# ml-rust/blazr

Hardware: NVIDIA B200
Metric: decode_tokens_per_s (higher is better)
Workload: dtype int8 activations x int4/6/8 weights, f64-exact accumulate -> f32

## Files before the change

### blazr_b200/csrc/formats.cuh

```cuda
#pragma once
#ifdef B200Q_HOST_CHECK
#include "hostcheck/host_shim.h"
#else
#include "common.cuh"
#endif
#ifdef __CUDACC__
#define IQ_TABLE_QUAL static __device__
#endif
#include "iq_grids.h"

namespace b200q {

struct Unit {
    uint32_t v[8];
    float a[2], b[2];
    int off[2];
};

template <class F, class = void>
struct FmtNoff { static constexpr int value = 0; };
template <class F>
struct FmtNoff<F, decltype((void)F::NOFF)> { static constexpr int value = F::NOFF; };

struct FmtMeta {
// ... 82 lines not shown
        u.a[0] = u.a[1] = __fmul_rn(d, (float)sc);
        u.b[0] = u.b[1] = __fmul_rn(dmin, (float)m);
        u.off[0] = u.off[1] = 0;
    }
#ifndef B200Q_HOST_CHECK
    static constexpr int NOFF = 5;
    __device__ __forceinline__ static void unit_offsets(int r0, int i, FmtMeta, uint32_t (&o)[NOFF]) {
        o[0] = QS + r0 * 128 + 16 * swz8(r0, i);
        o[1] = QS + (r0 + 4) * 128 + 16 * swz8(r0 + 4, i);
        o[2] = HDR + r0 * 16;
        o[3] = HDR + r0 * 16 + 4 + i;
        o[4] = HDR + r0 * 16 + 12 + (i >> 1);
    }
    template <int STEP>
    __device__ __forceinline__ static void load_unit_at(uint32_t c, const uint32_t (&o)[NOFF], int i, Unit& u, FmtMeta) {
        const uint4 w = lds128_sa(c + o[STEP]);
        const uint32_t dd = lds32_sa(c + o[2] + 64 * STEP);
        const uint32_t b1 = lds8_sa(c + o[3] + 64 * STEP), b2 = lds8_sa(c + o[4] + 64 * STEP);
        u.v[0] = w.x & 0x0F0F0F0Fu; u.v[1] = w.y & 0x0F0F0F0Fu; u.v[2] = w.z & 0x0F0F0F0Fu; u.v[3] = w.w & 0x0F0F0F0Fu;
        u.v[4] = w.x & 0xF0F0F0F0u; u.v[5] = w.y & 0xF0F0F0F0u; u.v[6] = w.z & 0xF0F0F0F0u; u.v[7] = w.w & 0xF0F0F0F0u;
        const float d = half_bits_to_float((uint16_t)(dd & 0xFFFF)), dmin = half_bits_to_float((uint16_t)(dd >> 16));
        const int sc = b1 & 63;
        const int m = (b1 >> 6) | (((b2 >> (4 * (i & 1))) & 0xF) << 2);
        u.a[0] = u.a[1] = __fmul_rn(d, (float)sc);
        u.b[0] = u.b[1] = __fmul_rn(dmin, (float)m);
        u.off[0] = u.off[1] = 0;
    }
#endif
};

struct FmtQ6K {
// ... 60 lines not shown
        u.b[0] = u.b[1] = 0.0f;
        u.off[0] = u.off[1] = 32;
    }
#ifndef B200Q_HOST_CHECK
    static constexpr int NOFF = 6;
    __device__ __forceinline__ static void unit_offsets(int r0, int i, FmtMeta, uint32_t (&o)[NOFF]) {
        o[0] = QL + r0 * 128 + 16 * swz8(r0, i);
        o[1] = QL + (r0 + 4) * 128 + 16 * swz8(r0 + 4, i);
        o[2] = QH + r0 * 64 + 16 * swz4(r0, i >> 1) + 8 * (i & 1);
        o[3] = QH + (r0 + 4) * 64 + 16 * swz4(r0 + 4, i >> 1) + 8 * (i & 1);
        o[4] = SC + r0 * 16 + 2 * i;
        o[5] = D + r0 * 2;
    }
    template <int STEP>
    __device__ __forceinline__ static void load_unit_at(uint32_t c, const uint32_t (&o)[NOFF], int, Unit& u, FmtMeta) {
        const uint4 w = lds128_sa(c + o[STEP]);
        const uint2 hq = lds64_sa(c + o[2 + STEP]);
        const uint32_t s2 = lds16_sa(c + o[4] + 64 * STEP);
        const float d = half_bits_to_float((uint16_t)lds16_sa(c + o[5] + 8 * STEP));
        const uint32_t M4 = 0x0F0F0F0Fu, MH = 0x30303030u;
        u.v[0] = (w.x & M4) | ((hq.x << 4) & MH);
        u.v[1] = (w.y & M4) | ((hq.x << 2) & MH);
        u.v[2] = (w.z & M4) | (hq.x & MH);
        u.v[3] = (w.w & M4) | ((hq.x >> 2) & MH);
        u.v[4] = ((w.x >> 4) & M4) | ((hq.y << 4) & MH);
        u.v[5] = ((w.y >> 4) & M4) | ((hq.y << 2) & MH);
        u.v[6] = ((w.z >> 4) & M4) | (hq.y & MH);
        u.v[7] = ((w.w >> 4) & M4) | ((hq.y >> 2) & MH);
        u.a[0] = __fmul_rn(d, (float)(int8_t)(s2 & 0xFF));
        u.a[1] = __fmul_rn(d, (float)(int8_t)(s2 >> 8));
        u.b[0] = u.b[1] = 0.0f;
        u.off[0] = u.off[1] = 32;
// ... 790 lines not shown
```

### blazr_b200/csrc/internal.h

```cpp
#pragma once
#include <cuda_runtime.h>
#include <stdint.h>

#include "../../include/b200q.h"

struct b200q_weight {
    int64_t N, K, N_pad, K_pad;
    int family, source, ggml_type, group_size, sub, gpc;
    int device;
    int chunk_bytes;
    int64_t T, KC;
    uint8_t* data;
    int64_t device_bytes, canonical_bytes;
    float* bias;
    int32_t* perm;
    int num_sms;
    const b200q_weight* next;
    const b200q_weight* pair;
};

struct b200q_bank {
    int E;
    b200q_weight proto;
    const uint8_t** table_dev;
// ... 8 lines not shown
                               cudaStream_t st);
cudaError_t launch_repack_awq(const uint32_t* qweight, const float* scales, const float* zeros, int64_t N_full, int64_t n0, int64_t k0,
                              const b200q_weight* w, int* err_flag, cudaStream_t st);
cudaError_t launch_repack_gptq(const uint32_t* qweight, const float* scales, const uint32_t* qzeros, const int32_t* perm, int zpo,
                               int64_t N_full, int64_t n0, int64_t k0, const b200q_weight* w, int* err_flag, cudaStream_t st);
cudaError_t launch_dequantize(const b200q_weight* w, void* out, int dtype, cudaStream_t st);
cudaError_t launch_act_quant(const void* x, int x_dtype, int64_t M, int64_t K, int64_t K_pad, int64_t ldx, const int32_t* perm, uint8_t* xq,
                             cudaStream_t st);
cudaError_t launch_act_unpack(const uint8_t* xq, int64_t M, int64_t K_pad, int8_t* q, float* d, int32_t* bsum16, cudaStream_t st);
cudaError_t launch_int_partials(const b200q_weight* w, const uint8_t* xq, int64_t M, int32_t* out, cudaStream_t st);
cudaError_t launch_to_bf16(const void* x, int x_dtype, int64_t M, int64_t K, int64_t K_pad, int64_t M_pad, int64_t ldx, const int32_t* perm,
                           void* out_bf16, cudaStream_t st);

struct MatvecPlan {
    int grid, nstages, stage_bytes, smem_bytes, mb, xhat_bytes;
};
struct FusedPrologue {
    int mode;
    const float* h_in;
    const float* delta;
    float* h_out;
    const float* norm_w;
    float eps;
    const float* gate_up;
};
cudaError_t matvec_plan(const b200q_weight* w, int64_t M, MatvecPlan* plan, int pro = 0);
size_t matvec_ws_bytes(const b200q_weight* w, int64_t M);
void set_matvec_trace(long long* dev_buf);
cudaError_t launch_l2_prefetch(const b200q_weight* w, int64_t M, int64_t max_bytes, cudaStream_t st);
struct RemoteOut;
// ... 19 lines not shown
```

### blazr_b200/csrc/matvec.cu

```cuda
#include <cstdlib>

#include "matvec_common.cuh"

namespace b200q {

__global__ void __launch_bounds__(32) l2_prefetch_kernel(const uint8_t* __restrict__ w, int64_t KC, int64_t C, int chunk_bytes, int first, int nchunks) {
    pdl_launch_dependents();
    if (threadIdx.x != 0) return;
    const int64_t G = gridDim.x, g = blockIdx.x;
    const int64_t c0 = sk_begin(g, C, G), c1 = sk_begin(g + 1, C, G);
    const SkPlan sp = sk_plan(c0, c1, KC);
    const int n = (int)(c1 - c0);
    const uint8_t* base = w + c0 * (int64_t)chunk_bytes;
    for (int j = first; j < n && j < first + nchunks; j++) {
        const uint8_t* src;
        if (j < sp.nH) src = base + (size_t)j * chunk_bytes;
        else if (j < sp.nH + sp.nT) src = base + (size_t)(sp.nH + sp.nF + (j - sp.nH)) * chunk_bytes;
        else src = base + (size_t)(sp.nH + (j - sp.nH - sp.nT)) * chunk_bytes;
        asm volatile("cp.async.bulk.prefetch.L2.global [%0], %1;" ::"l"(src), "r"(chunk_bytes) : "memory");
    }
}


static cudaError_t launch_family(int family, const MatvecParams& p, int mb, int grid, int smem, cudaStream_t st) {
// ... 26 lines not shown
    const int cbmax = (w2 && w2->chunk_bytes > w->chunk_bytes) ? w2->chunk_bytes : w->chunk_bytes;
    int stage = cbmax + (pro ? 0 : (int)M * ACT_REC_BYTES);
    stage = (stage + 127) & ~127;
    int xhat = pro ? (int)(((size_t)w->KC * M * ACT_REC_BYTES + 127) & ~(size_t)127) : 0;
    int budget_kb = 150;
    if (const char* e = getenv("B200Q_MV_SMEM_KB")) { int v = atoi(e); if (v >= 64 && v <= 214) budget_kb = v; }
    int budget = budget_kb * 1024 - MV_HDR_BYTES - xhat;
    int nst = budget / stage;
    if (nst > MV_MAX_STAGES) nst = MV_MAX_STAGES;
    if (const char* e = getenv("B200Q_MV_STAGES")) { int v = atoi(e); if (v >= 2 && v < nst) nst = v; }
    if (nst < 2) return cudaErrorInvalidValue;
    int64_t C = (w->T + (w2 ? w2->T : 0)) * w->KC;
    int64_t G = (int64_t)w->num_sms;
    if (const char* e = getenv("B200Q_MV_GRID")) { int v = atoi(e); if (v >= 1 && v <= w->num_sms) G = v; }
    if (G > C) G = C;
    plan->grid = (int)G;
    plan->nstages = nst;
    plan->stage_bytes = stage;
    plan->smem_bytes = MV_HDR_BYTES + xhat + nst * stage;
    plan->xhat_bytes = xhat;
    plan->mb = mb;
    return cudaSuccess;
}

size_t matvec_ws_bytes(const b200q_weight* w, int64_t M) {
    size_t cnt = ((size_t)w->T * 4 + 255) & ~(size_t)255;
    size_t part = (size_t)w->num_sms * 2 * TILE_ROWS * 4 * sizeof(double);
    (void)M;
    return cnt + part;
}
// ... 18 lines not shown
    p.M = (int)M;
    p.y_dtype = y_dtype;
    p.ldy = ldy;
    p.KC = w->KC;
    p.C = (w->T + (w2 ? w2->T : 0)) * w->KC;
    p.gpc = w->gpc;
    p.nstages = plan.nstages;
    p.chunk_bytes = (w2 && w2->chunk_bytes > w->chunk_bytes) ? w2->chunk_bytes : w->chunk_bytes;
    p.cb1 = w->chunk_bytes;
    p.cb2 = w2 ? w2->chunk_bytes : 0;
    p.w2 = w2 ? w2->data : nullptr;
    p.T1 = (int)w->T;
    p.gpc2 = w2 ? w2->gpc : 0;
    p.stage_bytes = plan.stage_bytes;
    p.pro = pro;
    p.xhat_bytes = plan.xhat_bytes;
    p.h_in = fp ? fp->h_in : nullptr;
    p.delta = fp ? fp->delta : nullptr;
    p.h_out = fp ? fp->h_out : nullptr;
    p.norm_w = fp ? fp->norm_w : nullptr;
    p.eps = fp ? fp->eps : 0.0f;
    p.gate_up = fp ? fp->gate_up : nullptr;
    p.w_table = nullptr;
    p.sel = nullptr;
    p.n_experts = 0;
    p.tpw = (int)(w->T + (w2 ? w2->T : 0));
    p.x_rows = (int)M;
    p.x_slot_div = 1;
    p.y_slot_stride = 0;
    p.trace = g_trace ? g_trace + (size_t)(g_trace_launch++) * 148 * 8 : nullptr;
// ... 56 lines not shown
    p.w = nullptr;
    p.xq = xq;
    p.y = y;
    p.bias = nullptr;
    size_t cnt = ((size_t)v.T * 4 + 255) & ~(size_t)255;
    p.ws_cnt = reinterpret_cast<unsigned int*>(ws);
    p.ws_part = reinterpret_cast<double*>(ws + cnt);
    p.N = b->proto.N;
    p.M = 1;
    p.y_dtype = y_dtype;
    p.ldy = b->proto.N;
    p.KC = v.KC;
    p.C = v.T * v.KC;
    p.gpc = v.gpc;
    p.nstages = plan.nstages;
    p.chunk_bytes = v.chunk_bytes;
    p.stage_bytes = plan.stage_bytes;
    p.w_table = b->table_dev;
    p.sel = sel_dev;
    p.n_experts = b->E;
    p.w2 = nullptr; p.cb1 = v.chunk_bytes; p.cb2 = 0; p.T1 = 0; p.gpc2 = 0;
    p.tpw = (int)b->proto.T;
    p.x_rows = (int)x_rows;
    p.x_slot_div = (int)x_slot_div;
    p.y_slot_stride = y_slot_stride;
    p.next_w = nullptr;
    p.next_pf = 0;
    p.xq_out = (uint8_t*)swiglu_xq_out;
    p.epi_F = (int)(b->proto.N / 2);
    p.epi_rows = (int)n_slots;
// ... 28 lines not shown
```

### blazr_b200/csrc/matvec_common.cuh

```cuda
#pragma once
#include "comm_dev.cuh"
#include "formats.cuh"
#include "internal.h"
#include "streamk_plan.cuh"

namespace b200q {


constexpr int MV_CONSUMER_WARPS = 16;
constexpr int MV_THREADS = (MV_CONSUMER_WARPS + 2) * 32;
constexpr int MV_ROWS_PER_WARP = TILE_ROWS / MV_CONSUMER_WARPS;
constexpr int MV_STEPS = MV_ROWS_PER_WARP / 4;
constexpr int MV_MAX_STAGES = 10;
constexpr int MV_HDR_BYTES = 256;

struct MatvecParams {
    const uint8_t* w;
    const uint8_t* xq;
    void* y;
    const float* bias;
    double* ws_part;
    unsigned int* ws_cnt;
    int64_t N;
    int M, y_dtype;
    int64_t ldy;
    int64_t KC, C;
    int gpc, nstages, chunk_bytes, stage_bytes;
// ... 13 lines not shown
    int next_chunk_bytes, next_G, next_pf;
    int rp_mode;
    CommDev comm;
    uint8_t* xq_out;
    int epi_F;
    int epi_rows;
    int plan32;
    const uint8_t* w2;
    int cb1, cb2, T1, gpc2;
    const uint8_t* const* w_table;
    const int32_t* sel;
    int n_experts;
    int tpw;
    int x_rows, x_slot_div;
    int64_t y_slot_stride;
};

template <int FAMILY>
cudaError_t mv_launch(const MatvecParams& p, int mb, int grid, int smem, cudaStream_t st);
cudaError_t mv_launch_dual_q4k_q6k(const MatvecParams& p, int mb, int grid, int smem, cudaStream_t st);

}
```

### blazr_b200/csrc/matvec_impl.cuh

```cuda
#pragma once
#include <atomic>
#include <type_traits>
#include "matvec_common.cuh"

namespace b200q {

__device__ __forceinline__ void quant_block_to_record(float v, uint8_t* rec, int blk_in_chunk, int lane) {
    float amax = fabsf(v);
#pragma unroll
    for (int o = 16; o > 0; o >>= 1) amax = fmaxf(amax, __shfl_xor_sync(0xffffffffu, amax, o));
    const float d = __fdiv_rn(amax, 127.0f);
    const float id = (d != 0.0f) ? __fdiv_rn(1.0f, d) : 0.0f;
    const int q = (int)roundf(__fmul_rn(v, id));
    int s = q;
#pragma unroll
    for (int o = 8; o > 0; o >>= 1) s += __shfl_xor_sync(0xffffffffu, s, o);
    const int s_hi = __shfl_sync(0xffffffffu, s, 16);
    rec[blk_in_chunk * 32 + lane] = (uint8_t)(int8_t)q;
    if (lane == 0) {
        reinterpret_cast<float*>(rec + 256)[blk_in_chunk] = d;
        reinterpret_cast<uint32_t*>(rec + 288)[blk_in_chunk] = ((uint32_t)s & 0xFFFFu) | ((uint32_t)s_hi << 16);
    }
}

// ... 173 lines not shown
    if constexpr (!RP) {
        store_out_d(p.y, p.y_dtype, idx, v);
    } else if (p.rp_mode == RP_ALLREDUCE) {
        const double e = ar_encode(v);
        for (int r = 0; r < p.comm.world; r++) reinterpret_cast<double*>(p.comm.peers[r] + rp.off)[idx] = e;
    } else {
        const float f = (float)v;
        for (int r = 0; r < p.comm.world; r++) reinterpret_cast<float*>(p.comm.peers[r] + rp.off)[idx] = f;
    }
}
template <bool RP>
__device__ __forceinline__ bool mv_use_bias(const MatvecParams& p) { return p.bias && (!RP || p.rp_mode != RP_ALLREDUCE || p.comm.rank == 0); }
constexpr int MV_BAR_DONE = 5;
constexpr int MV_BAR_EPI_FULL = 6;
constexpr int MV_BAR_EPI_FREE = 8;

enum { OUT_PLAIN = 0, OUT_REMOTE = 1 , OUT_SWIGLU = 2  };

__device__ __forceinline__ void swiglu_tile_epilogue(const MatvecParams& p, const float* sy , int64_t tile_in_weight, int rec_row, int lane) {
#pragma unroll
    for (int b = 0; b < 2; b++) {
        const int j = 32 * b + lane, w_ = j >> 2, g_ = j & 3;
        const float gv = sy[8 * w_ + g_], uv = sy[8 * w_ + 4 + g_];
        const float v = __fmul_rn(__fdiv_rn(gv, __fadd_rn(1.0f, det_expf(-gv))), uv);
        const int64_t f = 64 * tile_in_weight + 32 * b;
        if (f < p.epi_F) quant_block_to_record(v, p.xq_out + ((size_t)(f / CHUNK_K) * p.epi_rows + rec_row) * ACT_REC_BYTES, (int)((f % CHUNK_K) / 32), lane);
    }
}


__device__ __forceinline__ void sk_tile_span(const MatvecParams& p, int64_t tq, int64_t G, int& gf, int& gl, int& sgf) {
    if (p.plan32) {
        gf = (int)((((uint32_t)(tq * p.KC) + 1u) * (uint32_t)G - 1u) / (uint32_t)p.C);
        gl = (int)((((uint32_t)((tq + 1) * p.KC - 1) + 1u) * (uint32_t)G - 1u) / (uint32_t)p.C);
        sgf = ((int64_t)sk_begin32((uint32_t)gf, (uint32_t)p.C, (uint32_t)G) == tq * p.KC) ? 0 : 1;
    } else {
        gf = (int)sk_owner(tq * p.KC, p.C, G);
        gl = (int)sk_owner((tq + 1) * p.KC - 1, p.C, G);
        sgf = (sk_begin(gf, p.C, G) == tq * p.KC) ? 0 : 1;
    }
}
constexpr int MV_WIDE_MIN = 3;

template <class F, int MB, bool PRO, bool GRP, int OUT, class F2 = F>
__global__ void __launch_bounds__(MV_THREADS, 1) matvec_kernel(const MatvecParams p) {
    constexpr bool RP = OUT == OUT_REMOTE;
    constexpr bool EPI = OUT == OUT_SWIGLU;
    constexpr bool DUAL = !std::is_same<F, F2>::value;
    static_assert(!DUAL || (!GRP && OUT == OUT_PLAIN), "the dual-format launch is a plain matvec");
    __shared__ float s_y[EPI ? 2 : 1][EPI ? MB : 1][EPI ? TILE_ROWS : 1];
    __shared__ float s_yfix[EPI ? MB : 1][EPI ? TILE_ROWS : 1];
    extern __shared__ __align__(128) uint8_t smem[];
    uint64_t* full = reinterpret_cast<uint64_t*>(smem);
    uint64_t* empty = full + MV_MAX_STAGES;
    uint8_t* xhat = smem + MV_HDR_BYTES;
    uint8_t* stages = smem + MV_HDR_BYTES + (PRO ? p.xhat_bytes : 0);

    const int tid = threadIdx.x, warp = tid >> 5, lane = tid & 31;
    const int64_t G = gridDim.x, g = blockIdx.x;
    if (MV_TRACE_ON(p) && tid == 0) {
        p.trace[g * 8 + 0] = globaltimer_ns();
        unsigned smid;
        asm volatile("mov.u32 %0, %%smid;" : "=r"(smid));
        p.trace[g * 8 + 2] = smid;
    }
    int64_t c0, c1;
// ... 4 lines not shown
        c0 = sk_begin(g, p.C, G);
        c1 = sk_begin(g + 1, p.C, G);
    }
    const int n_chunks = (int)(c1 - c0);
    const int KC = (int)p.KC;
    const int nst = p.nstages;
    SkPlan& sp = *reinterpret_cast<SkPlan*>(smem + 2 * MV_MAX_STAGES * 8);
    pdl_launch_dependents();

    const bool is_producer = warp == MV_CONSUMER_WARPS && lane == 0;
    SkPlan spp;
    if (is_producer) {
        spp = p.plan32 ? sk_plan32((uint32_t)c0, (uint32_t)c1, (uint32_t)p.KC) : sk_plan(c0, c1, p.KC);
        for (int s = 0; s < nst; s++) {
            mbar_init(&full[s], 1);
            mbar_init(&empty[s], MV_CONSUMER_WARPS);
        }
        fence_mbar_init();
        fence_proxy_async();
        if (!GRP) {
            const uint64_t pol0 = policy_evict_first();
            const uint32_t xbytes0 = PRO ? 0u : (uint32_t)p.M * ACT_REC_BYTES;
            const int pre0 = n_chunks < nst ? n_chunks : nst;
            for (int j = 0; j < pre0; j++) {
                const int64_t vc0 = sk_chunk_at(spp, c0, j);
                const uint8_t* src0 = p.w + vc0 * (int64_t)p.cb1;
                uint32_t wb0 = (uint32_t)p.cb1;
                if (DUAL && vc0 >= (int64_t)p.T1 * p.KC) { src0 = p.w2 + (vc0 - (int64_t)p.T1 * p.KC) * (int64_t)p.cb2; wb0 = (uint32_t)p.cb2; }
                mbar_arrive_expect_tx(&full[j], wb0 + xbytes0);
                bulk_g2s_hint(stages + (size_t)j * p.stage_bytes, src0, wb0, &full[j], pol0);
            }
// ... 171 lines not shown
                const int buf = ft & 1;
                const int64_t tq = (int64_t)sp.tF + ft;
                named_bar_sync(MV_BAR_EPI_FULL + buf, MV_CONSUMER_WARPS * 32 + 32);
                for (int m = 0; m < p.M; m++) swiglu_tile_epilogue(p, s_y[buf][m], GRP ? tq % p.tpw : tq, GRP ? (int)(tq / p.tpw) : m, lane);
                __syncwarp();
                asm volatile("bar.arrive %0, %1;" ::"r"(MV_BAR_EPI_FREE + buf), "r"(MV_CONSUMER_WARPS * 32 + 32) : "memory");
            }
        }
        if (rp_on) named_bar_sync(MV_BAR_DONE, MV_CONSUMER_WARPS * 32 + 32);
        return;
    }

    if constexpr (!PRO) pdl_wait();
    RpState rp{0u, 0};
    if constexpr (RP) rp = rp_begin(p);
    const int g4 = lane >> 3, i = lane & 7;
    const FmtMeta meta{p.gpc};
    double acc[MV_STEPS][MB];
#pragma unroll
    for (int s4 = 0; s4 < MV_STEPS; s4++)
#pragma unroll
        for (int m = 0; m < MB; m++) acc[s4][m] = 0.0;

    if constexpr (PRO) {
        if (p.pro == 1) {
            __shared__ double s_red[MV_CONSUMER_WARPS];
            switch ((int)p.KC * CHUNK_K / (MV_CONSUMER_WARPS * 32)) {
                case 16: { float nw[16]; load_nw<16>(p.norm_w, tid, nw); pdl_wait_again(); norm_prologue<MB, 16>(p, xhat, nw, tid, warp, lane, g == 0, s_red); break; }
                case 8: { float nw[8]; load_nw<8>(p.norm_w, tid, nw); pdl_wait_again(); norm_prologue<MB, 8>(p, xhat, nw, tid, warp, lane, g == 0, s_red); break; }
                case 4: { float nw[4]; load_nw<4>(p.norm_w, tid, nw); pdl_wait_again(); norm_prologue<MB, 4>(p, xhat, nw, tid, warp, lane, g == 0, s_red); break; }
                case 2: { float nw[2]; load_nw<2>(p.norm_w, tid, nw); pdl_wait_again(); norm_prologue<MB, 2>(p, xhat, nw, tid, warp, lane, g == 0, s_red); break; }
                default: { float nw[1]; load_nw<1>(p.norm_w, tid, nw); pdl_wait_again(); norm_prologue<MB, 1>(p, xhat, nw, tid, warp, lane, g == 0, s_red); break; }
            }
        } else {
            pdl_wait_again();
            fused_prologue<MB>(p, xhat, tid, warp, lane, g == 0);
        }
    }

    bool wide_reducer = false;
    int wide_gf = 0, wide_gl = 0, wide_sgf = 0;
    if (sp.nH > 0) {
        sk_tile_span(p, sp.tH, G, wide_gf, wide_gl, wide_sgf);
        wide_reducer = (wide_gl - wide_gf + 1) >= MV_WIDE_MIN && (int)g == wide_gf + 1;
    }
    int kcur = sp.nH > 0 ? sp.kcH : 0;
    int seg = sp.nH > 0 ? 0 : (sp.nT > 0 ? 1 : 2);
    int seg_left = seg == 0 ? sp.nH : (seg == 1 ? sp.nT : KC);
    int t = seg == 0 ? sp.tH : (seg == 1 ? sp.tT : sp.tF);
    int s = 0;
    uint32_t ph = 0;
    int n_full_done = 0;
    constexpr int NOFF = FmtNoff<F>::value;
    const uint32_t stages_sa = smem_u32(stages), full_sa = keep_in_reg(smem_u32(full)), xhat_sa = smem_u32(xhat);
    constexpr uint32_t EMPTY_OFF = MV_MAX_STAGES * 8;
    const uint32_t ring_bytes = (uint32_t)nst * (uint32_t)p.stage_bytes;
    uint32_t st_off = 0;
    uint32_t bar_sa = full_sa;
    uint32_t uoff[NOFF > 0 ? NOFF : 1];
    if constexpr (NOFF > 0) {
        F::unit_offsets(MV_ROWS_PER_WARP * warp + g4, i, meta, uoff);
#pragma unroll
        for (int q = 0; q < NOFF; q++) uoff[q] = keep_in_reg(uoff[q] + stages_sa);
    }
    constexpr int NOFF2 = DUAL ? FmtNoff<F2>::value : 0;
    const FmtMeta meta2{p.gpc2};
    uint32_t uoff2[NOFF2 > 0 ? NOFF2 : 1];
    if constexpr (NOFF2 > 0) {
        F2::unit_offsets(MV_ROWS_PER_WARP * warp + g4, i, meta2, uoff2);
#pragma unroll
        for (int q = 0; q < NOFF2; q++) uoff2[q] = keep_in_reg(uoff2[q] + stages_sa);
    }
    const uint32_t xq_off = keep_in_reg((PRO ? xhat_sa : stages_sa + (uint32_t)p.chunk_bytes) + 32u * (uint32_t)i);
    const uint32_t xs_off = keep_in_reg((PRO ? xhat_sa : stages_sa + (uint32_t)p.chunk_bytes) + 256u + 4u * (uint32_t)i);
    const uint32_t xrec_step = (uint32_t)p.M * ACT_REC_BYTES;
    uint32_t xk_off = PRO ? (uint32_t)kcur * xrec_step : 0u;
    for (int j = 0; j < n_chunks; j++) {
        mbar_wait_sa(bar_sa, ph);
        if (MV_TRACE_ON(p) && tid == 0 && j == 0) p.trace[g * 8 + 1] = globaltimer_ns();
        const uint8_t* wc = stages + (size_t)s * p.stage_bytes;
        const uint32_t xbase = PRO ? xk_off : st_off;
        if (PRO) { xk_off += xrec_step; if (++kcur == KC) { kcur = 0; xk_off = 0u; } }

        uint4 xa[MB], xb[MB];
        float dx[MB];
        int bsA[MB], bsB[MB];
#pragma unroll
        for (int m = 0; m < MB; m++) {
            xa[m] = lds128_sa(xq_off + xbase + m * ACT_REC_BYTES);
            xb[m] = lds128_sa(xq_off + xbase + m * ACT_REC_BYTES + 16);
            dx[m] = __uint_as_float(lds32_sa(xs_off + xbase + m * ACT_REC_BYTES));
            const uint32_t bs = lds32_sa(xs_off + xbase + m * ACT_REC_BYTES + 32);
            bsA[m] = (int)(int16_t)(bs & 0xFFFFu);
            bsB[m] = (int)(int16_t)(bs >> 16);
        }
        const bool skip_chunk = GRP && *reinterpret_cast<const volatile int*>(wc + p.chunk_bytes + p.M * ACT_REC_BYTES) != 0;
        auto chunk_math = [&](auto tag, const auto& uo, const FmtMeta& mt) {
            using FF = decltype(tag);
            constexpr int NO = FmtNoff<FF>::value;
#pragma unroll
            for (int s4 = 0; s4 < MV_STEPS; s4++) {
                Unit u;
                if constexpr (NO > 0) {
                    if (s4 == 0) FF::template load_unit_at<0>(st_off, uo, i, u, mt);
                    else FF::template load_unit_at<1>(st_off, uo, i, u, mt);
                } else {
                    const int r = MV_ROWS_PER_WARP * warp + 4 * s4 + g4;
                    FF::template load_unit<true, FF::NIB>(wc, r, i, u, mt);
                }
#pragma unroll
                for (int m = 0; m < MB; m++) {
                    int sA = 0, sB = 0;
                    sA = __dp4a((int)u.v[0], (int)xa[m].x, sA); sA = __dp4a((int)u.v[1], (int)xa[m].y, sA);
                    sA = __dp4a((int)u.v[2], (int)xa[m].z, sA); sA = __dp4a((int)u.v[3], (int)xa[m].w, sA);
                    if constexpr (FF::NIB) {
                        sB = dp4a_us(u.v[4], xb[m].x, sB); sB = dp4a_us(u.v[5], xb[m].y, sB);
                        sB = dp4a_us(u.v[6], xb[m].z, sB); sB = dp4a_us(u.v[7], xb[m].w, sB);
                        sB >>= 4;
                    } else {
                        sB = __dp4a((int)u.v[4], (int)xb[m].x, sB); sB = __dp4a((int)u.v[5], (int)xb[m].y, sB);
                        sB = __dp4a((int)u.v[6], (int)xb[m].z, sB); sB = __dp4a((int)u.v[7], (int)xb[m].w, sB);
                    }
                    sA -= u.off[0] * bsA[m];
                    sB -= u.off[1] * bsB[m];
                    double a_ = acc[s4][m];
                    if (FF::SUB == 32) {
                        a_ = fma((double)__fmul_rn(u.a[0], dx[m]), i2d(sA + sB), a_);
                        if (FF::HAS_MIN) a_ = fma(-(double)__fmul_rn(u.b[0], dx[m]), i2d(bsA[m] + bsB[m]), a_);
                    } else {
                        a_ = fma((double)__fmul_rn(u.a[0], dx[m]), i2d(sA), a_);
                        if (FF::HAS_MIN) a_ = fma(-(double)__fmul_rn(u.b[0], dx[m]), i2d(bsA[m]), a_);
                        a_ = fma((double)__fmul_rn(u.a[1], dx[m]), i2d(sB), a_);
                        if (FF::HAS_MIN) a_ = fma(-(double)__fmul_rn(u.b[1], dx[m]), i2d(bsB[m]), a_);
                    }
                    acc[s4][m] = a_;
                }
            }
        };
        if (!MV_DEBUG_SKIP(p) && !skip_chunk) {
            if constexpr (DUAL) {
                if (t >= p.T1) chunk_math(F2{}, uoff2, meta2);
                else chunk_math(F{}, uoff, meta);
            } else {
                chunk_math(F{}, uoff, meta);
            }
        }
        __syncwarp();
        if (lane == 0) mbar_arrive_sa(bar_sa + EMPTY_OFF);
        st_off += (uint32_t)p.stage_bytes;
        bar_sa += 8u;
        ++s;
        if (st_off == ring_bytes) { s = 0; ph ^= 1u; st_off = 0u; bar_sa = full_sa; }

        if (--seg_left > 0) continue;

#pragma unroll
        for (int s4 = 0; s4 < MV_STEPS; s4++)
#pragma unroll
            for (int m = 0; m < MB; m++) {
                double v = acc[s4][m];
                v += __shfl_xor_sync(0xffffffffu, v, 1);
                v += __shfl_xor_sync(0xffffffffu, v, 2);
                v += __shfl_xor_sync(0xffffffffu, v, 4);
                acc[s4][m] = v;
            }
        if (EPI && seg == 2) {
            const int buf = n_full_done & 1;
            if (n_full_done >= 2) named_bar_sync(MV_BAR_EPI_FREE + buf, MV_CONSUMER_WARPS * 32 + 32);
            if (i == 0) {
                const int64_t tl = GRP ? t % p.tpw : t;
#pragma unroll
                for (int s4 = 0; s4 < MV_STEPS; s4++) {
                    const int rr = MV_ROWS_PER_WARP * warp + 4 * s4 + g4;
                    const int64_t n = tl * TILE_ROWS + rr;
                    const double bv = (p.bias && n < p.N) ? (double)p.bias[n] : 0.0;
#pragma unroll
                    for (int m = 0; m < MB; m++) s_y[buf][m][rr] = (float)(acc[s4][m] + bv);
                }
                __threadfence_block();
            }
            __syncwarp();
            asm volatile("bar.arrive %0, %1;" ::"r"(MV_BAR_EPI_FULL + buf), "r"(MV_CONSUMER_WARPS * 32 + 32) : "memory");
            n_full_done++;
        } else if (seg == 2) {
            if (i == 0) {
#pragma unroll
                const int64_t tl = GRP ? t % p.tpw : t;
                const int64_t ybase = GRP ? (int64_t)(t / p.tpw) * p.y_slot_stride : 0;
                for (int s4 = 0; s4 < MV_STEPS; s4++) {
                    const int64_t n = tl * TILE_ROWS + MV_ROWS_PER_WARP * warp + 4 * s4 + g4;
                    if (n < p.N) {
                        const double bv = mv_use_bias<RP>(p) ? (double)p.bias[n] : 0.0;
#pragma unroll
                        for (int m = 0; m < MB; m++)
                            if (m < p.M) mv_store<RP>(p, rp, ybase + (int64_t)m * p.ldy + n, acc[s4][m] + bv);
                    }
                }
            }
        } else {
            double* part = p.ws_part + ((size_t)g * 2 + seg) * (TILE_ROWS * MB);
            if (i == 0) {
#pragma unroll
                for (int s4 = 0; s4 < MV_STEPS; s4++) {
                    const int rr = MV_ROWS_PER_WARP * warp + 4 * s4 + g4;
#pragma unroll
                    for (int m = 0; m < MB; m++) {
                        const double v = acc[s4][m];
                        asm volatile("st.volatile.global.f64 [%0], %1;" ::"l"(part + rr * MB + m), "d"(v == 0.0 ? -0.0 : v) : "memory");
                    }
                }
            }
            if (seg == 0 && wide_reducer) {
                constexpr int NT = MV_CONSUMER_WARPS * 32;
                constexpr int PASSES = 2 * MB;
                named_bar_sync(4, NT);
                if (MV_TRACE_ON(p) && tid == 0) p.trace[g * 8 + 5] = globaltimer_ns();
                double* red = reinterpret_cast<double*>(stages);
                int wpr = (int)(ring_bytes / (uint32_t)(TILE_ROWS * MB * 8));
                if (wpr > MV_CONSUMER_WARPS) wpr = MV_CONSUMER_WARPS;
// ... 34 lines not shown
                    if constexpr (EPI) {
                        if (m < p.M) s_yfix[m][rr] = (float)(sv + ((p.bias && n < p.N) ? (double)p.bias[n] : 0.0));
                    } else {
                        if (n < p.N && m < p.M) mv_store<RP>(p, rp, ybase + (int64_t)m * p.ldy + n, sv + (mv_use_bias<RP>(p) ? (double)p.bias[n] : 0.0));
                    }
                }
                if constexpr (EPI) {
                    named_bar_sync(4, NT);
                    if (warp == 0)
                        for (int m = 0; m < p.M; m++) swiglu_tile_epilogue(p, s_yfix[m], tql, GRP ? (int)(t / p.tpw) : m, lane);
                }
                if (MV_TRACE_ON(p) && tid == 0) p.trace[g * 8 + 7] = globaltimer_ns();
            }
        }
#pragma unroll
        for (int s4 = 0; s4 < MV_STEPS; s4++)
#pragma unroll
            for (int m = 0; m < MB; m++) acc[s4][m] = 0.0;

        if (seg == 0 && sp.nT > 0) { seg = 1; seg_left = sp.nT; t = sp.tT; kcur = 0; xk_off = 0u; }
        else if (seg != 2) { seg = 2; seg_left = KC; t = sp.tF; kcur = 0; xk_off = 0u; }
        else { seg_left = KC; t++; }

    }
    if constexpr (RP) {
        named_bar_sync(MV_BAR_DONE, MV_CONSUMER_WARPS * 32 + 32);
        if (tid == 0) {
            uint8_t* mine = p.comm.peers[p.comm.rank];
            if (p.rp_mode == RP_ALLREDUCE) {
                ar_epoch_arrive(mine, rp.epoch, (unsigned int)G);
            } else {
                unsigned int* done = reinterpret_cast<unsigned int*>(mine + COMM_OFF_AG_DONE);
                asm volatile("fence.acq_rel.sys;" ::: "memory");
                unsigned int old;
                asm volatile("atom.acq_rel.gpu.global.add.u32 %0, [%1], 1;" : "=r"(old) : "l"(done) : "memory");
                if (old == (unsigned int)(G - 1)) {
                    *done = 0u;
                    comm_raise_flags(p.comm, COMM_OFF_AG_FLAGS, 0, rp.epoch);
                    *reinterpret_cast<unsigned int*>(mine + COMM_OFF_AG_EPOCH) = rp.epoch;
                }
            }
        }
    }
    if (MV_TRACE_ON(p) && tid == 0) p.trace[g * 8 + 3] = globaltimer_ns();
}

template <class F, int MB, bool PRO, bool GRP, int OUT = OUT_PLAIN, class F2 = F>
static cudaError_t launch_t(const MatvecParams& p, int grid, int smem, cudaStream_t st) {
    static std::atomic<bool> configured[16];
    int dev = 0;
    cudaGetDevice(&dev);
    if (dev >= 16 || !configured[dev].load(std::memory_order_acquire)) {
        cudaError_t e = cudaFuncSetAttribute(matvec_kernel<F, MB, PRO, GRP, OUT, F2>, cudaFuncAttributeMaxDynamicSharedMemorySize, 216 * 1024);
        if (e != cudaSuccess) return e;
        if (dev < 16) configured[dev].store(true, std::memory_order_release);
    }
    cudaLaunchConfig_t cfg = {};
    cfg.gridDim = dim3((unsigned)grid);
    cfg.blockDim = dim3(MV_THREADS);
    cfg.dynamicSmemBytes = (size_t)smem;
    cfg.stream = st;
    cudaLaunchAttribute attr[1];
    attr[0].id = cudaLaunchAttributeProgrammaticStreamSerialization;
    attr[0].val.programmaticStreamSerializationAllowed = 1;
    cfg.attrs = attr;
    cfg.numAttrs = 1;
    cudaError_t le = cudaLaunchKernelEx(&cfg, matvec_kernel<F, MB, PRO, GRP, OUT, F2>, p);
    if (le != cudaSuccess) return le;
    count_launch();
    return cudaGetLastError();
}

template <class F, class F2>
static cudaError_t launch_dual(const MatvecParams& p, int mb, int grid, int smem, cudaStream_t st) {
    if (p.w_table || p.rp_mode != RP_NONE || p.xq_out || !p.w2) return cudaErrorInvalidValue;
    switch (mb) {
        case 1: return p.pro ? launch_t<F, 1, true, false, OUT_PLAIN, F2>(p, grid, smem, st) : launch_t<F, 1, false, false, OUT_PLAIN, F2>(p, grid, smem, st);
        case 2: return p.pro ? launch_t<F, 2, true, false, OUT_PLAIN, F2>(p, grid, smem, st) : launch_t<F, 2, false, false, OUT_PLAIN, F2>(p, grid, smem, st);
        case 4: return p.pro ? launch_t<F, 4, true, false, OUT_PLAIN, F2>(p, grid, smem, st) : launch_t<F, 4, false, false, OUT_PLAIN, F2>(p, grid, smem, st);
        default: return cudaErrorInvalidValue;
    }
}

template <class F>
static cudaError_t launch_f(const MatvecParams& p, int mb, int grid, int smem, cudaStream_t st) {
    if (p.w_table) {
        if (mb != 1 || p.pro || p.rp_mode) return cudaErrorInvalidValue;
        return p.xq_out ? launch_t<F, 1, false, true, OUT_SWIGLU>(p, grid, smem, st) : launch_t<F, 1, false, true>(p, grid, smem, st);
    }
    if (p.rp_mode != RP_NONE) {
        if (p.pro || p.xq_out) return cudaErrorInvalidValue;
        switch (mb) {
            case 1: return launch_t<F, 1, false, false, OUT_REMOTE>(p, grid, smem, st);
            case 2: return launch_t<F, 2, false, false, OUT_REMOTE>(p, grid, smem, st);
            case 4: return launch_t<F, 4, false, false, OUT_REMOTE>(p, grid, smem, st);
            default: return cudaErrorInvalidValue;
        }
    }
    if (p.xq_out) {
        switch (mb) {
            case 1: return p.pro ? launch_t<F, 1, true, false, OUT_SWIGLU>(p, grid, smem, st) : launch_t<F, 1, false, false, OUT_SWIGLU>(p, grid, smem, st);
            case 2: return p.pro ? launch_t<F, 2, true, false, OUT_SWIGLU>(p, grid, smem, st) : launch_t<F, 2, false, false, OUT_SWIGLU>(p, grid, smem, st);
            case 4: return p.pro ? launch_t<F, 4, true, false, OUT_SWIGLU>(p, grid, smem, st) : launch_t<F, 4, false, false, OUT_SWIGLU>(p, grid, smem, st);
// ... 14 lines not shown
```

Measured before the change: 114.2.

## Split consumer warps into two chunk groups for Q4_K matvec at M=1

For Q4_K weights at batch 1 with enough chunks per block, the consumer warps are split into two groups. Each group handles alternate pipeline stages and covers twice as many rows per warp, and the two groups' partial sums are combined through shared memory behind a named barrier at each segment flush. The aim is more chunks in flight and better latency hiding in the decode matvec. In exchange it adds more per-warp registers and accumulators, an extra barrier per tile flush, and an even stage count.

```diff
diff --git a/blazr_b200/csrc/formats.cuh b/blazr_b200/csrc/formats.cuh
--- a/blazr_b200/csrc/formats.cuh
+++ b/blazr_b200/csrc/formats.cuh
@@ -120,7 +120,7 @@
     }
     template <int STEP>
     __device__ __forceinline__ static void load_unit_at(uint32_t c, const uint32_t (&o)[NOFF], int i, Unit& u, FmtMeta) {
-        const uint4 w = lds128_sa(c + o[STEP]);
+        const uint4 w = lds128_sa(c + o[STEP & 1] + (STEP >> 1) * 8 * 128);
         const uint32_t dd = lds32_sa(c + o[2] + 64 * STEP);
         const uint32_t b1 = lds8_sa(c + o[3] + 64 * STEP), b2 = lds8_sa(c + o[4] + 64 * STEP);
         u.v[0] = w.x & 0x0F0F0F0Fu; u.v[1] = w.y & 0x0F0F0F0Fu; u.v[2] = w.z & 0x0F0F0F0Fu; u.v[3] = w.w & 0x0F0F0F0Fu;
@@ -211,8 +211,8 @@
     }
     template <int STEP>
     __device__ __forceinline__ static void load_unit_at(uint32_t c, const uint32_t (&o)[NOFF], int, Unit& u, FmtMeta) {
-        const uint4 w = lds128_sa(c + o[STEP]);
-        const uint2 hq = lds64_sa(c + o[2 + STEP]);
+        const uint4 w = lds128_sa(c + o[STEP & 1] + (STEP >> 1) * 8 * 128);
+        const uint2 hq = lds64_sa(c + o[2 + (STEP & 1)] + (STEP >> 1) * 8 * 64);
         const uint32_t s2 = lds16_sa(c + o[4] + 64 * STEP);
         const float d = half_bits_to_float((uint16_t)lds16_sa(c + o[5] + 8 * STEP));
         const uint32_t M4 = 0x0F0F0F0Fu, MH = 0x30303030u;
diff --git a/blazr_b200/csrc/internal.h b/blazr_b200/csrc/internal.h
--- a/blazr_b200/csrc/internal.h
+++ b/blazr_b200/csrc/internal.h
@@ -46,6 +46,7 @@
 
 struct MatvecPlan {
     int grid, nstages, stage_bytes, smem_bytes, mb, xhat_bytes;
+    int groups;
 };
 struct FusedPrologue {
     int mode;
diff --git a/blazr_b200/csrc/matvec.cu b/blazr_b200/csrc/matvec.cu
--- a/blazr_b200/csrc/matvec.cu
+++ b/blazr_b200/csrc/matvec.cu
@@ -64,6 +64,9 @@
     int64_t G = (int64_t)w->num_sms;
     if (const char* e = getenv("B200Q_MV_GRID")) { int v = atoi(e); if (v >= 1 && v <= w->num_sms) G = v; }
     if (G > C) G = C;
+    const int groups = (mb == 1 && w->family == B200Q_FAM_Q4_K && C >= (int64_t)MV_GROUP_MIN_CHUNKS * G) ? 2 : 1;
+    if (groups > 1 && (nst & 1)) nst -= 1;
+    plan->groups = groups;
     plan->grid = (int)G;
     plan->nstages = nst;
     plan->stage_bytes = stage;
@@ -112,6 +115,7 @@
     p.gpc2 = w2 ? w2->gpc : 0;
     p.stage_bytes = plan.stage_bytes;
     p.pro = pro;
+    p.groups = plan.groups;
     p.xhat_bytes = plan.xhat_bytes;
     p.h_in = fp ? fp->h_in : nullptr;
     p.delta = fp ? fp->delta : nullptr;
@@ -198,6 +202,7 @@
     p.C = v.T * v.KC;
     p.gpc = v.gpc;
     p.nstages = plan.nstages;
+    p.groups = plan.groups;
     p.chunk_bytes = v.chunk_bytes;
     p.stage_bytes = plan.stage_bytes;
     p.w_table = b->table_dev;
diff --git a/blazr_b200/csrc/matvec_common.cuh b/blazr_b200/csrc/matvec_common.cuh
--- a/blazr_b200/csrc/matvec_common.cuh
+++ b/blazr_b200/csrc/matvec_common.cuh
@@ -11,6 +11,7 @@
 constexpr int MV_THREADS = (MV_CONSUMER_WARPS + 2) * 32;
 constexpr int MV_ROWS_PER_WARP = TILE_ROWS / MV_CONSUMER_WARPS;
 constexpr int MV_STEPS = MV_ROWS_PER_WARP / 4;
+constexpr int MV_GROUP_MIN_CHUNKS = 8;
 constexpr int MV_MAX_STAGES = 10;
 constexpr int MV_HDR_BYTES = 256;
 
@@ -54,6 +55,7 @@
     int tpw;
     int x_rows, x_slot_div;
     int64_t y_slot_stride;
+    int groups;
 };
 
 template <int FAMILY>
diff --git a/blazr_b200/csrc/matvec_impl.cuh b/blazr_b200/csrc/matvec_impl.cuh
--- a/blazr_b200/csrc/matvec_impl.cuh
+++ b/blazr_b200/csrc/matvec_impl.cuh
@@ -1,6 +1,7 @@
 #pragma once
 #include <atomic>
 #include <type_traits>
+#include <utility>
 #include "matvec_common.cuh"
 
 namespace b200q {
@@ -211,6 +212,13 @@
 constexpr int MV_BAR_DONE = 5;
 constexpr int MV_BAR_EPI_FULL = 6;
 constexpr int MV_BAR_EPI_FREE = 8;
+template <class Fn, int... I>
+__device__ __forceinline__ void mv_static_for_impl(Fn&& fn, std::integer_sequence<int, I...>) { (fn(std::integral_constant<int, I>{}), ...); }
+template <int N, class Fn>
+__device__ __forceinline__ void mv_static_for(Fn&& fn) { mv_static_for_impl(fn, std::make_integer_sequence<int, N>{}); }
+constexpr int MV_BAR_COMB = 10;
+template <class F>
+constexpr bool mv_has_groups() { return std::is_same<F, FmtQ4K>::value; }
 
 enum { OUT_PLAIN = 0, OUT_REMOTE = 1 , OUT_SWIGLU = 2  };
 
@@ -239,7 +247,7 @@
 }
 constexpr int MV_WIDE_MIN = 3;
 
-template <class F, int MB, bool PRO, bool GRP, int OUT, class F2 = F>
+template <class F, int MB, bool PRO, bool GRP, int OUT, class F2 = F, int NG = 1>
 __global__ void __launch_bounds__(MV_THREADS, 1) matvec_kernel(const MatvecParams p) {
     constexpr bool RP = OUT == OUT_REMOTE;
     constexpr bool EPI = OUT == OUT_SWIGLU;
@@ -247,6 +255,7 @@
     static_assert(!DUAL || (!GRP && OUT == OUT_PLAIN), "the dual-format launch is a plain matvec");
     __shared__ float s_y[EPI ? 2 : 1][EPI ? MB : 1][EPI ? TILE_ROWS : 1];
     __shared__ float s_yfix[EPI ? MB : 1][EPI ? TILE_ROWS : 1];
+    __shared__ double s_comb[NG > 1 ? 2 : 1][NG > 1 ? TILE_ROWS * MB : 1];
     extern __shared__ __align__(128) uint8_t smem[];
     uint64_t* full = reinterpret_cast<uint64_t*>(smem);
     uint64_t* empty = full + MV_MAX_STAGES;
@@ -281,7 +290,7 @@
         spp = p.plan32 ? sk_plan32((uint32_t)c0, (uint32_t)c1, (uint32_t)p.KC) : sk_plan(c0, c1, p.KC);
         for (int s = 0; s < nst; s++) {
             mbar_init(&full[s], 1);
-            mbar_init(&empty[s], MV_CONSUMER_WARPS);
+            mbar_init(&empty[s], MV_CONSUMER_WARPS / NG);
         }
         fence_mbar_init();
         fence_proxy_async();
@@ -483,11 +492,18 @@
     if constexpr (!PRO) pdl_wait();
     RpState rp{0u, 0};
     if constexpr (RP) rp = rp_begin(p);
+    constexpr int GW = MV_CONSUMER_WARPS / NG;
+    constexpr int RPW = TILE_ROWS / GW;
+    constexpr int STEPS = RPW / 4;
+    static_assert((NG == 1 || NG == 2) && (NG == 1 || MB == 1), "groups: 1, or 2 at M = 1 (register budget)");
+    const int grp = warp / GW;
     const int g4 = lane >> 3, i = lane & 7;
+    const int r0 = RPW * (warp % GW) + g4;
+    const bool writer = grp == 0 && i == 0;
     const FmtMeta meta{p.gpc};
-    double acc[MV_STEPS][MB];
-#pragma unroll
-    for (int s4 = 0; s4 < MV_STEPS; s4++)
+    double acc[STEPS][MB];
+#pragma unroll
+    for (int s4 = 0; s4 < STEPS; s4++)
 #pragma unroll
         for (int m = 0; m < MB; m++) acc[s4][m] = 0.0;
 
@@ -513,22 +529,23 @@
         sk_tile_span(p, sp.tH, G, wide_gf, wide_gl, wide_sgf);
         wide_reducer = (wide_gl - wide_gf + 1) >= MV_WIDE_MIN && (int)g == wide_gf + 1;
     }
-    int kcur = sp.nH > 0 ? sp.kcH : 0;
+    int kc0 = sp.nH > 0 ? sp.kcH : 0;
     int seg = sp.nH > 0 ? 0 : (sp.nT > 0 ? 1 : 2);
-    int seg_left = seg == 0 ? sp.nH : (seg == 1 ? sp.nT : KC);
+    int seg_len = seg == 0 ? sp.nH : (seg == 1 ? sp.nT : KC);
     int t = seg == 0 ? sp.tH : (seg == 1 ? sp.tT : sp.tF);
-    int s = 0;
     uint32_t ph = 0;
     int n_full_done = 0;
+    int n_flush = 0;
     constexpr int NOFF = FmtNoff<F>::value;
     const uint32_t stages_sa = smem_u32(stages), full_sa = keep_in_reg(smem_u32(full)), xhat_sa = smem_u32(xhat);
     constexpr uint32_t EMPTY_OFF = MV_MAX_STAGES * 8;
     const uint32_t ring_bytes = (uint32_t)nst * (uint32_t)p.stage_bytes;
-    uint32_t st_off = 0;
-    uint32_t bar_sa = full_sa;
+    const uint32_t ring_step = (uint32_t)NG * (uint32_t)p.stage_bytes;
+    uint32_t st_off = (uint32_t)grp * (uint32_t)p.stage_bytes;
+    uint32_t bar_sa = full_sa + 8u * (uint32_t)grp;
     uint32_t uoff[NOFF > 0 ? NOFF : 1];
     if constexpr (NOFF > 0) {
-        F::unit_offsets(MV_ROWS_PER_WARP * warp + g4, i, meta, uoff);
+        F::unit_offsets(r0, i, meta, uoff);
 #pragma unroll
         for (int q = 0; q < NOFF; q++) uoff[q] = keep_in_reg(uoff[q] + stages_sa);
     }
@@ -536,95 +553,95 @@
     const FmtMeta meta2{p.gpc2};
     uint32_t uoff2[NOFF2 > 0 ? NOFF2 : 1];
     if constexpr (NOFF2 > 0) {
-        F2::unit_offsets(MV_ROWS_PER_WARP * warp + g4, i, meta2, uoff2);
+        F2::unit_offsets(r0, i, meta2, uoff2);
 #pragma unroll
         for (int q = 0; q < NOFF2; q++) uoff2[q] = keep_in_reg(uoff2[q] + stages_sa);
     }
     const uint32_t xq_off = keep_in_reg((PRO ? xhat_sa : stages_sa + (uint32_t)p.chunk_bytes) + 32u * (uint32_t)i);
     const uint32_t xs_off = keep_in_reg((PRO ? xhat_sa : stages_sa + (uint32_t)p.chunk_bytes) + 256u + 4u * (uint32_t)i);
     const uint32_t xrec_step = (uint32_t)p.M * ACT_REC_BYTES;
-    uint32_t xk_off = PRO ? (uint32_t)kcur * xrec_step : 0u;
-    for (int j = 0; j < n_chunks; j++) {
-        mbar_wait_sa(bar_sa, ph);
-        if (MV_TRACE_ON(p) && tid == 0 && j == 0) p.trace[g * 8 + 1] = globaltimer_ns();
-        const uint8_t* wc = stages + (size_t)s * p.stage_bytes;
-        const uint32_t xbase = PRO ? xk_off : st_off;
-        if (PRO) { xk_off += xrec_step; if (++kcur == KC) { kcur = 0; xk_off = 0u; } }
-
-        uint4 xa[MB], xb[MB];
-        float dx[MB];
-        int bsA[MB], bsB[MB];
-#pragma unroll
-        for (int m = 0; m < MB; m++) {
-            xa[m] = lds128_sa(xq_off + xbase + m * ACT_REC_BYTES);
-            xb[m] = lds128_sa(xq_off + xbase + m * ACT_REC_BYTES + 16);
-            dx[m] = __uint_as_float(lds32_sa(xs_off + xbase + m * ACT_REC_BYTES));
-            const uint32_t bs = lds32_sa(xs_off + xbase + m * ACT_REC_BYTES + 32);
-            bsA[m] = (int)(int16_t)(bs & 0xFFFFu);
-            bsB[m] = (int)(int16_t)(bs >> 16);
-        }
-        const bool skip_chunk = GRP && *reinterpret_cast<const volatile int*>(wc + p.chunk_bytes + p.M * ACT_REC_BYTES) != 0;
-        auto chunk_math = [&](auto tag, const auto& uo, const FmtMeta& mt) {
-            using FF = decltype(tag);
-            constexpr int NO = FmtNoff<FF>::value;
-#pragma unroll
-            for (int s4 = 0; s4 < MV_STEPS; s4++) {
-                Unit u;
-                if constexpr (NO > 0) {
-                    if (s4 == 0) FF::template load_unit_at<0>(st_off, uo, i, u, mt);
-                    else FF::template load_unit_at<1>(st_off, uo, i, u, mt);
+    for (int jb = 0; jb < n_chunks; ) {
+        const int je = jb + seg_len;
+        int j = jb + ((grp - jb) & (NG - 1));
+        uint32_t xk_off = PRO ? (uint32_t)(kc0 + j - jb) * xrec_step : 0u;
+        for (; j < je; j += NG) {
+            mbar_wait_sa(bar_sa, ph);
+            if (MV_TRACE_ON(p) && tid == 0 && j == 0) p.trace[g * 8 + 1] = globaltimer_ns();
+            const uint8_t* wc = stages + st_off;
+            const uint32_t xbase = PRO ? xk_off : st_off;
+            if (PRO) xk_off += (uint32_t)NG * xrec_step;
+
+            uint4 xa[MB], xb[MB];
+            float dx[MB];
+            int bsA[MB], bsB[MB];
+#pragma unroll
+            for (int m = 0; m < MB; m++) {
+                xa[m] = lds128_sa(xq_off + xbase + m * ACT_REC_BYTES);
+                xb[m] = lds128_sa(xq_off + xbase + m * ACT_REC_BYTES + 16);
+                dx[m] = __uint_as_float(lds32_sa(xs_off + xbase + m * ACT_REC_BYTES));
+                const uint32_t bs = lds32_sa(xs_off + xbase + m * ACT_REC_BYTES + 32);
+                bsA[m] = (int)(int16_t)(bs & 0xFFFFu);
+                bsB[m] = (int)(int16_t)(bs >> 16);
+            }
+            const bool skip_chunk = GRP && *reinterpret_cast<const volatile int*>(wc + p.chunk_bytes + p.M * ACT_REC_BYTES) != 0;
+            auto chunk_math = [&](auto tag, const auto& uo, const FmtMeta& mt) {
+                using FF = decltype(tag);
+                constexpr int NO = FmtNoff<FF>::value;
+                mv_static_for<STEPS>([&](auto step) {
+                    constexpr int s4 = decltype(step)::value;
+                    Unit u;
+                    if constexpr (NO > 0) {
+                        FF::template load_unit_at<s4>(st_off, uo, i, u, mt);
+                    } else {
+                        FF::template load_unit<true, FF::NIB>(wc, r0 + 4 * s4, i, u, mt);
+                    }
+#pragma unroll
+                    for (int m = 0; m < MB; m++) {
+                        int sA = 0, sB = 0;
+                        sA = __dp4a((int)u.v[0], (int)xa[m].x, sA); sA = __dp4a((int)u.v[1], (int)xa[m].y, sA);
+                        sA = __dp4a((int)u.v[2], (int)xa[m].z, sA); sA = __dp4a((int)u.v[3], (int)xa[m].w, sA);
+                        if constexpr (FF::NIB) {
+                            sB = dp4a_us(u.v[4], xb[m].x, sB); sB = dp4a_us(u.v[5], xb[m].y, sB);
+                            sB = dp4a_us(u.v[6], xb[m].z, sB); sB = dp4a_us(u.v[7], xb[m].w, sB);
+                            sB >>= 4;
+                        } else {
+                            sB = __dp4a((int)u.v[4], (int)xb[m].x, sB); sB = __dp4a((int)u.v[5], (int)xb[m].y, sB);
+                            sB = __dp4a((int)u.v[6], (int)xb[m].z, sB); sB = __dp4a((int)u.v[7], (int)xb[m].w, sB);
+                        }
+                        sA -= u.off[0] * bsA[m];
+                        sB -= u.off[1] * bsB[m];
+                        double a_ = acc[s4][m];
+                        if (FF::SUB == 32) {
+                            a_ = fma((double)__fmul_rn(u.a[0], dx[m]), i2d(sA + sB), a_);
+                            if (FF::HAS_MIN) a_ = fma(-(double)__fmul_rn(u.b[0], dx[m]), i2d(bsA[m] + bsB[m]), a_);
+                        } else {
+                            a_ = fma((double)__fmul_rn(u.a[0], dx[m]), i2d(sA), a_);
+                            if (FF::HAS_MIN) a_ = fma(-(double)__fmul_rn(u.b[0], dx[m]), i2d(bsA[m]), a_);
+                            a_ = fma((double)__fmul_rn(u.a[1], dx[m]), i2d(sB), a_);
+                            if (FF::HAS_MIN) a_ = fma(-(double)__fmul_rn(u.b[1], dx[m]), i2d(bsB[m]), a_);
+                        }
+                        acc[s4][m] = a_;
+                    }
+                });
+            };
+            if (!MV_DEBUG_SKIP(p) && !skip_chunk) {
+                if constexpr (DUAL) {
+                    if (t >= p.T1) chunk_math(F2{}, uoff2, meta2);
+                    else chunk_math(F{}, uoff, meta);
                 } else {
-                    const int r = MV_ROWS_PER_WARP * warp + 4 * s4 + g4;
-                    FF::template load_unit<true, FF::NIB>(wc, r, i, u, mt);
-                }
-#pragma unroll
-                for (int m = 0; m < MB; m++) {
-                    int sA = 0, sB = 0;
-                    sA = __dp4a((int)u.v[0], (int)xa[m].x, sA); sA = __dp4a((int)u.v[1], (int)xa[m].y, sA);
-                    sA = __dp4a((int)u.v[2], (int)xa[m].z, sA); sA = __dp4a((int)u.v[3], (int)xa[m].w, sA);
-                    if constexpr (FF::NIB) {
-                        sB = dp4a_us(u.v[4], xb[m].x, sB); sB = dp4a_us(u.v[5], xb[m].y, sB);
-                        sB = dp4a_us(u.v[6], xb[m].z, sB); sB = dp4a_us(u.v[7], xb[m].w, sB);
-                        sB >>= 4;
-                    } else {
-                        sB = __dp4a((int)u.v[4], (int)xb[m].x, sB); sB = __dp4a((int)u.v[5], (int)xb[m].y, sB);
-                        sB = __dp4a((int)u.v[6], (int)xb[m].z, sB); sB = __dp4a((int)u.v[7], (int)xb[m].w, sB);
-                    }
-                    sA -= u.off[0] * bsA[m];
-                    sB -= u.off[1] * bsB[m];
-                    double a_ = acc[s4][m];
-                    if (FF::SUB == 32) {
-                        a_ = fma((double)__fmul_rn(u.a[0], dx[m]), i2d(sA + sB), a_);
-                        if (FF::HAS_MIN) a_ = fma(-(double)__fmul_rn(u.b[0], dx[m]), i2d(bsA[m] + bsB[m]), a_);
-                    } else {
-                        a_ = fma((double)__fmul_rn(u.a[0], dx[m]), i2d(sA), a_);
-                        if (FF::HAS_MIN) a_ = fma(-(double)__fmul_rn(u.b[0], dx[m]), i2d(bsA[m]), a_);
-                        a_ = fma((double)__fmul_rn(u.a[1], dx[m]), i2d(sB), a_);
-                        if (FF::HAS_MIN) a_ = fma(-(double)__fmul_rn(u.b[1], dx[m]), i2d(bsB[m]), a_);
-                    }
-                    acc[s4][m] = a_;
-                }
-            }
-        };
-        if (!MV_DEBUG_SKIP(p) && !skip_chunk) {
-            if constexpr (DUAL) {
-                if (t >= p.T1) chunk_math(F2{}, uoff2, meta2);
-                else chunk_math(F{}, uoff, meta);
-            } else {
-                chunk_math(F{}, uoff, meta);
-            }
-        }
-        __syncwarp();
-        if (lane == 0) mbar_arrive_sa(bar_sa + EMPTY_OFF);
-        st_off += (uint32_t)p.stage_bytes;
-        bar_sa += 8u;
-        ++s;
-        if (st_off == ring_bytes) { s = 0; ph ^= 1u; st_off = 0u; bar_sa = full_sa; }
-
-        if (--seg_left > 0) continue;
-
-#pragma unroll
-        for (int s4 = 0; s4 < MV_STEPS; s4++)
+                    chunk_math(F{}, uoff, meta);
+                }
+            }
+            __syncwarp();
+            if (lane == 0) mbar_arrive_sa(bar_sa + EMPTY_OFF);
+            st_off += ring_step;
+            bar_sa += 8u * NG;
+            if (st_off >= ring_bytes) { ph ^= 1u; st_off -= ring_bytes; bar_sa -= 8u * (uint32_t)nst; }
+        }
+        jb = je;
+
+#pragma unroll
+        for (int s4 = 0; s4 < STEPS; s4++)
 #pragma unroll
             for (int m = 0; m < MB; m++) {
                 double v = acc[s4][m];
@@ -633,14 +650,31 @@
                 v += __shfl_xor_sync(0xffffffffu, v, 4);
                 acc[s4][m] = v;
             }
+        if constexpr (NG > 1) {
+            double* cb = s_comb[n_flush & 1];
+            if (grp == 1 && i == 0) {
+#pragma unroll
+                for (int s4 = 0; s4 < STEPS; s4++)
+#pragma unroll
+                    for (int m = 0; m < MB; m++) cb[(r0 + 4 * s4) * MB + m] = acc[s4][m];
+            }
+            named_bar_sync(MV_BAR_COMB, MV_CONSUMER_WARPS * 32);
+            if (writer) {
+#pragma unroll
+                for (int s4 = 0; s4 < STEPS; s4++)
+#pragma unroll
+                    for (int m = 0; m < MB; m++) acc[s4][m] += cb[(r0 + 4 * s4) * MB + m];
+            }
+            n_flush++;
+        }
         if (EPI && seg == 2) {
             const int buf = n_full_done & 1;
             if (n_full_done >= 2) named_bar_sync(MV_BAR_EPI_FREE + buf, MV_CONSUMER_WARPS * 32 + 32);
-            if (i == 0) {
+            if (writer) {
                 const int64_t tl = GRP ? t % p.tpw : t;
 #pragma unroll
-                for (int s4 = 0; s4 < MV_STEPS; s4++) {
-                    const int rr = MV_ROWS_PER_WARP * warp + 4 * s4 + g4;
+                for (int s4 = 0; s4 < STEPS; s4++) {
+                    const int rr = r0 + 4 * s4;
                     const int64_t n = tl * TILE_ROWS + rr;
                     const double bv = (p.bias && n < p.N) ? (double)p.bias[n] : 0.0;
 #pragma unroll
@@ -652,12 +686,12 @@
             asm volatile("bar.arrive %0, %1;" ::"r"(MV_BAR_EPI_FULL + buf), "r"(MV_CONSUMER_WARPS * 32 + 32) : "memory");
             n_full_done++;
         } else if (seg == 2) {
-            if (i == 0) {
-#pragma unroll
+            if (writer) {
                 const int64_t tl = GRP ? t % p.tpw : t;
                 const int64_t ybase = GRP ? (int64_t)(t / p.tpw) * p.y_slot_stride : 0;
-                for (int s4 = 0; s4 < MV_STEPS; s4++) {
-                    const int64_t n = tl * TILE_ROWS + MV_ROWS_PER_WARP * warp + 4 * s4 + g4;
+#pragma unroll
+                for (int s4 = 0; s4 < STEPS; s4++) {
+                    const int64_t n = tl * TILE_ROWS + r0 + 4 * s4;
                     if (n < p.N) {
                         const double bv = mv_use_bias<RP>(p) ? (double)p.bias[n] : 0.0;
 #pragma unroll
@@ -668,10 +702,10 @@
             }
         } else {
             double* part = p.ws_part + ((size_t)g * 2 + seg) * (TILE_ROWS * MB);
-            if (i == 0) {
-#pragma unroll
-                for (int s4 = 0; s4 < MV_STEPS; s4++) {
-                    const int rr = MV_ROWS_PER_WARP * warp + 4 * s4 + g4;
+            if (writer) {
+#pragma unroll
+                for (int s4 = 0; s4 < STEPS; s4++) {
+                    const int rr = r0 + 4 * s4;
 #pragma unroll
                     for (int m = 0; m < MB; m++) {
                         const double v = acc[s4][m];
@@ -736,14 +770,13 @@
             }
         }
 #pragma unroll
-        for (int s4 = 0; s4 < MV_STEPS; s4++)
+        for (int s4 = 0; s4 < STEPS; s4++)
 #pragma unroll
             for (int m = 0; m < MB; m++) acc[s4][m] = 0.0;
 
-        if (seg == 0 && sp.nT > 0) { seg = 1; seg_left = sp.nT; t = sp.tT; kcur = 0; xk_off = 0u; }
-        else if (seg != 2) { seg = 2; seg_left = KC; t = sp.tF; kcur = 0; xk_off = 0u; }
-        else { seg_left = KC; t++; }
-
+        if (seg == 0 && sp.nT > 0) { seg = 1; seg_len = sp.nT; t = sp.tT; kc0 = 0; }
+        else if (seg != 2) { seg = 2; seg_len = KC; t = sp.tF; kc0 = 0; }
+        else { seg_len = KC; t++; }
     }
     if constexpr (RP) {
         named_bar_sync(MV_BAR_DONE, MV_CONSUMER_WARPS * 32 + 32);
@@ -767,13 +800,13 @@
     if (MV_TRACE_ON(p) && tid == 0) p.trace[g * 8 + 3] = globaltimer_ns();
 }
 
-template <class F, int MB, bool PRO, bool GRP, int OUT = OUT_PLAIN, class F2 = F>
+template <class F, int MB, bool PRO, bool GRP, int OUT = OUT_PLAIN, class F2 = F, int NG = 1>
 static cudaError_t launch_t(const MatvecParams& p, int grid, int smem, cudaStream_t st) {
     static std::atomic<bool> configured[16];
     int dev = 0;
     cudaGetDevice(&dev);
     if (dev >= 16 || !configured[dev].load(std::memory_order_acquire)) {
-        cudaError_t e = cudaFuncSetAttribute(matvec_kernel<F, MB, PRO, GRP, OUT, F2>, cudaFuncAttributeMaxDynamicSharedMemorySize, 216 * 1024);
+        cudaError_t e = cudaFuncSetAttribute(matvec_kernel<F, MB, PRO, GRP, OUT, F2, NG>, cudaFuncAttributeMaxDynamicSharedMemorySize, 216 * 1024);
         if (e != cudaSuccess) return e;
         if (dev < 16) configured[dev].store(true, std::memory_order_release);
     }
@@ -787,7 +820,7 @@
     attr[0].val.programmaticStreamSerializationAllowed = 1;
     cfg.attrs = attr;
     cfg.numAttrs = 1;
-    cudaError_t le = cudaLaunchKernelEx(&cfg, matvec_kernel<F, MB, PRO, GRP, OUT, F2>, p);
+    cudaError_t le = cudaLaunchKernelEx(&cfg, matvec_kernel<F, MB, PRO, GRP, OUT, F2, NG>, p);
     if (le != cudaSuccess) return le;
     count_launch();
     return cudaGetLastError();
@@ -796,6 +829,10 @@
 template <class F, class F2>
 static cudaError_t launch_dual(const MatvecParams& p, int mb, int grid, int smem, cudaStream_t st) {
     if (p.w_table || p.rp_mode != RP_NONE || p.xq_out || !p.w2) return cudaErrorInvalidValue;
+    if constexpr (mv_has_groups<F>()) {
+        if (mb == 1 && p.groups == 2)
+            return p.pro ? launch_t<F, 1, true, false, OUT_PLAIN, F2, 2>(p, grid, smem, st) : launch_t<F, 1, false, false, OUT_PLAIN, F2, 2>(p, grid, smem, st);
+    }
     switch (mb) {
         case 1: return p.pro ? launch_t<F, 1, true, false, OUT_PLAIN, F2>(p, grid, smem, st) : launch_t<F, 1, false, false, OUT_PLAIN, F2>(p, grid, smem, st);
         case 2: return p.pro ? launch_t<F, 2, true, false, OUT_PLAIN, F2>(p, grid, smem, st) : launch_t<F, 2, false, false, OUT_PLAIN, F2>(p, grid, smem, st);
@@ -808,7 +845,17 @@
 static cudaError_t launch_f(const MatvecParams& p, int mb, int grid, int smem, cudaStream_t st) {
     if (p.w_table) {
         if (mb != 1 || p.pro || p.rp_mode) return cudaErrorInvalidValue;
+        if constexpr (mv_has_groups<F>())
+            if (p.groups == 2)
+                return p.xq_out ? launch_t<F, 1, false, true, OUT_SWIGLU, F, 2>(p, grid, smem, st) : launch_t<F, 1, false, true, OUT_PLAIN, F, 2>(p, grid, smem, st);
         return p.xq_out ? launch_t<F, 1, false, true, OUT_SWIGLU>(p, grid, smem, st) : launch_t<F, 1, false, true>(p, grid, smem, st);
+    }
+    if constexpr (mv_has_groups<F>()) {
+        if (mb == 1 && p.groups == 2) {
+            if (p.rp_mode != RP_NONE) return (p.pro || p.xq_out) ? cudaErrorInvalidValue : launch_t<F, 1, false, false, OUT_REMOTE, F, 2>(p, grid, smem, st);
+            if (p.xq_out) return p.pro ? launch_t<F, 1, true, false, OUT_SWIGLU, F, 2>(p, grid, smem, st) : launch_t<F, 1, false, false, OUT_SWIGLU, F, 2>(p, grid, smem, st);
+            return p.pro ? launch_t<F, 1, true, false, OUT_PLAIN, F, 2>(p, grid, smem, st) : launch_t<F, 1, false, false, OUT_PLAIN, F, 2>(p, grid, smem, st);
+        }
     }
     if (p.rp_mode != RP_NONE) {
         if (p.pro || p.xq_out) return cudaErrorInvalidValue;
```

After: 116.8 (median of 6 runs). +2.2%, better.
